# lukecavabarrett/pna

Hardware: NVIDIA H100
Metric: aggregated edges/sec (PNA layer fwd) (higher is better)
Workload: dtype f32

## Files before the change

include/pna_b200.h:

```cpp
#ifndef PNA_B200_H
#define PNA_B200_H

#include <stddef.h>
#include <stdint.h>

#ifdef __cplusplus
extern "C" {
#endif

#define PNA_ABI_VERSION 8

typedef void* pna_stream_t;

enum pna_status {
  PNA_OK = 0,
  PNA_ERR_BAD_ARG = -1,
  PNA_ERR_UNSUPPORTED = -2,
  PNA_ERR_CUDA = -3,
  PNA_ERR_INDEX = -4,
  PNA_ERR_WORKSPACE = -5
};

enum pna_dtype { PNA_F32 = 0, PNA_BF16 = 1 };

enum pna_aggr { PNA_AGGR_SUM = 0, PNA_AGGR_MEAN = 1, PNA_AGGR_MIN = 2, PNA_AGGR_MAX = 3, PNA_AGGR_VAR = 4, PNA_AGGR_STD = 5,
                PNA_AGGR_SKIP = 15  };
enum pna_scaler { PNA_SCALE_IDENTITY = 0, PNA_SCALE_AMPLIFICATION = 1, PNA_SCALE_ATTENUATION = 2, PNA_SCALE_LINEAR = 3, PNA_SCALE_INVERSE_LINEAR = 4 };

#define PNA_MAX_AGGR 6
#define PNA_MAX_SCALERS 5

enum pna_flags {
  PNA_FLAG_ZERO_ISOLATED = 1u,
  PNA_FLAG_SKIP_LIGHT = 2u,
  PNA_FLAG_SKIP_HUBS = 4u,
  PNA_FLAG_GATHER_L1 = 16u,
  PNA_FLAG_RELU_VAR = 8u
};

enum pna_query_what {
  PNA_QUERY_ABI_VERSION = 0,
  PNA_QUERY_SM_ARCH = 1,
  PNA_QUERY_DEFAULT_SPLIT = 2,
  PNA_QUERY_DEFAULT_CHUNK = 3,
  PNA_QUERY_DEVICE_SM_COUNT = 4,
  PNA_QUERY_MAX_FEATURES = 5,
  PNA_QUERY_SIZEOF_CSR = 6,
  PNA_QUERY_SIZEOF_AGG = 7
};

typedef struct pna_csr {
  int64_t n_nodes;
  int64_t n_edges;
  int32_t split_threshold;
  int32_t chunk_edges;
  int32_t* rowptr;
  int32_t* col;
  int32_t* perm;
  int32_t* hub_info;
  int32_t* chunk_items;
  int64_t cap_hubs;
  int64_t cap_chunks;
  int64_t n_hubs;
  int64_t n_chunks;
  int32_t max_degree;
  int32_t n_part;
  int32_t* light_rowptr;
  int32_t* light_deg;
  int32_t* light_col;
  int32_t* part;
// ... 108 lines not shown
```

pna_b200/_lib.py:

```python
from __future__ import annotations

import ctypes as C
import os
import subprocess
import threading

_HERE = os.path.dirname(os.path.abspath(__file__))
REPO_ROOT = os.path.dirname(_HERE)
LIB_PATH = os.environ.get("PNA_B200_LIB") or os.path.join(_HERE, "libpna_sm90.so")
CUDA_SOURCES = [os.path.join(_HERE, "csrc", n) for n in
                ("pna_aggregate.cu", "pna_aggregate_f32_vec.cu", "pna_aggregate_f32_scalar.cu", "pna_aggregate_bf16_vec.cu",
                 "pna_aggregate_bf16_scalar.cu", "pna_aggregate_f32_fsplit.cu", "pna_aggregate_bwd.cu", "pna_linear.cu", "pna_csr.cu", "pna_peer.cu", "pna_misc.cu")]
CUDA_HEADERS = [os.path.join(_HERE, "csrc", n) for n in ("common.cuh", "pna_aggregate.cuh", "pna_aggregate_impl.cuh")] + [
    os.path.join(REPO_ROOT, "include", "pna_b200.h")]
BUILD_DIR = os.path.join(_HERE, "csrc", "build")

NVCC_FLAGS = ["-gencode", "arch=compute_90a,code=sm_90a", "-lineinfo", "-O3", "-std=c++17", "-fmad=false", "-Xcompiler", "-fPIC"]

ABI_VERSION = 8
PNA_OK = 0
PNA_F32, PNA_BF16 = 0, 1
AGGR_CODES = {"sum": 0, "mean": 1, "min": 2, "max": 3, "var": 4, "std": 5, "_skip": 15}
SCALER_CODES = {"identity": 0, "amplification": 1, "attenuation": 2, "linear": 3, "inverse_linear": 4}
FLAG_ZERO_ISOLATED, FLAG_SKIP_LIGHT, FLAG_SKIP_HUBS, FLAG_RELU_VAR, FLAG_GATHER_L1 = 1, 2, 4, 8, 16
(QUERY_ABI_VERSION, QUERY_SM_ARCH, QUERY_DEFAULT_SPLIT, QUERY_DEFAULT_CHUNK, QUERY_DEVICE_SM_COUNT,
 QUERY_MAX_FEATURES, QUERY_SIZEOF_CSR, QUERY_SIZEOF_AGG) = range(8)

EXPORTED_SYMBOLS = ("pna_csr_workspace_bytes", "pna_csr_build", "pna_csr_light_view", "pna_csr_light_view_workspace_bytes", "pna_aggregate_fwd", "pna_aggregate_bwd",
                    "pna_aggregate_bwd_coef", "pna_aggregate_bwd_combine", "pna_aggregate_bwd_slots",
                    "pna_gather_rows", "pna_halo_pull", "pna_halo_grad_pull", "pna_peer_barrier", "pna_linear_fwd", "pna_linear_scaled_fwd", "pna_row_scales", "pna_linear_workspace_bytes", "pna_query", "pna_last_error")


class PnaError(RuntimeError):

    def __init__(self, status: int, message: str):
        super().__init__(f"libpna_sm90 status {status}: {message}")
        self.status = status


class CsrStruct(C.Structure):
    _fields_ = [
        ("n_nodes", C.c_int64), ("n_edges", C.c_int64),
        ("split_threshold", C.c_int32), ("chunk_edges", C.c_int32),
        ("rowptr", C.c_void_p), ("col", C.c_void_p), ("perm", C.c_void_p),
        ("hub_info", C.c_void_p), ("chunk_items", C.c_void_p),
        ("cap_hubs", C.c_int64), ("cap_chunks", C.c_int64),
        ("n_hubs", C.c_int64), ("n_chunks", C.c_int64),
        ("max_degree", C.c_int32), ("n_part", C.c_int32),
        ("light_rowptr", C.c_void_p), ("light_deg", C.c_void_p), ("light_col", C.c_void_p), ("part", C.c_void_p),
        ("n_light_edges", C.c_int64), ("n_src_nodes", C.c_int64), ("hot_source_fraction", C.c_float), ("reserved", C.c_int32),
    ]


class AggStruct(C.Structure):
    _fields_ = [
        ("gathered", C.c_void_p), ("ld_gathered", C.c_int64),
        ("rowptr", C.c_void_p), ("col", C.c_void_p),
# ... 149 lines not shown
```

pna_b200/aggregate.py:

```python
from __future__ import annotations

import ctypes as C
import os
from typing import Mapping, Optional, Sequence, Union

import torch

from . import _lib
from .csr import CSRGraph

_DTYPES = {torch.float32: _lib.PNA_F32, torch.bfloat16: _lib.PNA_BF16}
Names = Union[str, Sequence[str]]


def _names(v: Names) -> list:
    return v.split() if isinstance(v, str) else list(v)


def _ptr(t: Optional[torch.Tensor]):
    return None if t is None else t.data_ptr()


def _rows2d(t: torch.Tensor, what: str) -> torch.Tensor:
    if t.dim() != 2:
        raise ValueError(f"{what} must be 2-D, got shape {tuple(t.shape)}")
    if t.size(1) > 1 and t.stride(1) != 1:
        t = t.contiguous()
    if t.size(0) > 1 and t.stride(0) < t.size(1):
        t = t.contiguous()
    return t


HOT_SOURCE_FRACTION_FOR_L1 = 0.25


DYNAMIC_TAIL_MIN_PARTITION_COST = 256


def _dynamic_tail(csr: CSRGraph) -> bool:
    env = os.environ.get("PNA_B200_DYNAMIC_TAIL")
    if env is not None:
        return env != "0"
    return csr.n_part > 0 and (csr.n_edges + 12 * csr.n_nodes) / csr.n_part >= DYNAMIC_TAIL_MIN_PARTITION_COST


def _check_scaler_degree(t: torch.Tensor, n_rows: int, dev) -> torch.Tensor:
    if t.dtype != torch.int32 or t.device != dev or t.numel() != n_rows or not t.is_contiguous():
        raise ValueError("scaler_degree must be a contiguous int32 [n_rows] tensor on the same device")
    return t


def fold_finalize_enabled() -> bool:
    return os.environ.get("PNA_B200_FOLD_FINALIZE", "0") == "1"


def output_width(n_feat: int, n_aggr: int, n_scalers: int, has_self: bool) -> int:
    return (n_aggr * n_scalers + (1 if has_self else 0)) * n_feat


def aggregate_forward(gathered: torch.Tensor, csr: CSRGraph, aggregators: Names, scalers: Names,
                      avg_deg: Mapping[str, float], *, towers: int = 1, row_bias: Optional[torch.Tensor] = None,
                      self_feat: Optional[torch.Tensor] = None, self_divided: bool = True,
                      messages_in_csr_order: bool = False, zero_isolated: bool = False, relu_var: bool = False,
                      out: Optional[torch.Tensor] = None, row_ids: Optional[torch.Tensor] = None,
                      skip_light: bool = False, skip_hubs: bool = False, view=None, peer=None,
                      scaler_degree: Optional[torch.Tensor] = None, gather_l1: Optional[bool] = None) -> torch.Tensor:
    if not gathered.is_cuda:
        raise ValueError("pna_b200 kernels run on CUDA tensors only; there is no CPU fallback")
    if gathered.dtype not in _DTYPES:
        raise TypeError(f"unsupported dtype {gathered.dtype}; libpna_sm90 takes float32 and bfloat16")
    dev = gathered.device
    if csr.device != dev:
        raise ValueError(f"CSR lives on {csr.device}, features on {dev}")
    gathered = _rows2d(gathered, "gathered")
    F = int(gathered.size(1))
    N = csr.n_nodes
    if F % towers != 0:
        raise ValueError(f"feature width {F} not divisible by towers={towers}")
    Ft = F // towers
    if messages_in_csr_order:
        if gathered.size(0) != csr.n_edges:
            raise ValueError("messages_in_csr_order needs one row per CSR slot")
    n_aggr, aggr_codes = _lib.pack_codes(aggregators, _lib.AGGR_CODES, "aggregator")
    n_scal, scal_codes = _lib.pack_codes(scalers, _lib.SCALER_CODES, "scaler")
    if row_bias is not None:
        row_bias = _rows2d(row_bias.to(gathered.dtype), "row_bias")
        if tuple(row_bias.shape) != (N, F):
            raise ValueError(f"row_bias must be [{N}, {F}]")
    if self_feat is not None:
        self_feat = _rows2d(self_feat.to(gathered.dtype), "self_feat")
        need = F if self_divided else Ft
        if self_feat.size(0) != N or self_feat.size(1) != need:
            raise ValueError(f"self_feat must be [{N}, {need}]")
    width = towers * output_width(Ft, n_aggr, n_scal, self_feat is not None)
    if out is None:
        out = torch.empty((N, width), dtype=gathered.dtype, device=dev)
    else:
        if out.dtype != gathered.dtype or out.device != dev or out.dim() != 2 or out.size(0) != N or out.size(1) < width \
                or out.stride(1) != 1:
            raise ValueError("bad `out` buffer")
    if row_ids is not None:
        if row_ids.dtype != torch.int32 or not row_ids.is_contiguous() or row_ids.device != dev:
            raise ValueError("row_ids must be a contiguous int32 tensor on the same device")
    if gather_l1 is None:
        gather_l1 = (not messages_in_csr_order) and peer is None and csr.hot_source_fraction > HOT_SOURCE_FRACTION_FOR_L1
    flags = (_lib.FLAG_GATHER_L1 if gather_l1 else 0) | \
            (_lib.FLAG_ZERO_ISOLATED if zero_isolated else 0) | (_lib.FLAG_SKIP_LIGHT if skip_light else 0) | \
            (_lib.FLAG_SKIP_HUBS if skip_hubs else 0) | (_lib.FLAG_RELU_VAR if relu_var else 0)
    partials = None if skip_hubs else csr.hub_partials(F)
    d = _lib.AggStruct(
        gathered=_ptr(gathered), ld_gathered=gathered.stride(0) if gathered.size(0) > 1 else F,
        rowptr=_ptr(csr.rowptr), col=None if messages_in_csr_order else (_ptr(csr.col) if csr.n_edges else None),
        row_bias=_ptr(row_bias), ld_row_bias=0 if row_bias is None else (row_bias.stride(0) if N > 1 else F),
        self_feat=_ptr(self_feat), ld_self=0 if self_feat is None else (self_feat.stride(0) if N > 1 else self_feat.size(1)),
        self_tower_stride=Ft if (self_feat is not None and self_divided) else 0,
        out=_ptr(out), ld_out=out.stride(0) if N > 1 else out.size(1),
        n_rows=N, n_feat=F, n_towers=towers, dtype=_DTYPES[gathered.dtype],
        n_aggr=n_aggr, aggr_codes=aggr_codes, n_scalers=n_scal, scaler_codes=scal_codes,
        avg_log=float(avg_deg["log"]), avg_lin=float(avg_deg.get("lin", 1.0)),
        flags=flags, split_threshold=csr.split_threshold, chunk_edges=csr.chunk_edges,
        hub_info=_ptr(csr.hub_info) if csr.n_hubs else None, chunk_items=_ptr(csr.chunk_items) if csr.n_hubs else None,
        n_hubs=csr.n_hubs, n_chunks=csr.n_chunks, hub_partials=_ptr(partials), max_degree=int(csr.max_degree),
        row_ids=_ptr(row_ids), n_row_ids=0 if row_ids is None else int(row_ids.numel()))
    if scaler_degree is not None:
        d.scaler_degree = _check_scaler_degree(scaler_degree, N, dev).data_ptr()
    if view is None and row_ids is None and _dynamic_tail(csr):
        d.work_counter = _ptr(csr.work_counter())
    if view is None and row_ids is None:
        view = csr.full_view()
        if fold_finalize_enabled() and not skip_hubs and peer is None:
            d.hub_done = _ptr(csr.hub_done())
    if view is not None and row_ids is None and N > 0:
        d.light_rowptr, d.light_deg, d.part, d.n_part = _ptr(view.light_rowptr), _ptr(view.light_deg), _ptr(view.part), view.n_part
        d.light_col = _ptr(view.light_col) if csr.n_edges else None
        d.n_view_rows = view.n_view_rows or N
    if peer is not None:
        ptr_table, shift = peer
        if ptr_table.dtype != torch.int64 or ptr_table.device != dev:
            raise ValueError("peer pointer table must be an int64 tensor on the same device")
# ... 186 lines not shown
```

pna_b200/csrc/pna_aggregate_f32_fsplit.cu:

```cuda
#include "pna_aggregate_impl.cuh"

namespace pna {

template <typename Cfg>
static int launch_fsplit(const KParams& p_in, cudaStream_t st) {
  constexpr int VEC = 2, K = 1, DEPTH = 1;
  KParams p = p_in;
  p.n_fpass = (p.F + 32 * VEC * K - 1) / (32 * VEC * K);
  p.work_ctr = nullptr;
  constexpr size_t smem = StreamGeom<float, VEC, K, DEPTH>::kSmem;
  auto kern = k_rows_stream<float, VEC, K, Cfg, false, DEPTH, false>;
  static int resident = 0;
  if (resident == 0) {
    if (smem > 48 * 1024) PNA_CUDA_TRY(cudaFuncSetAttribute(kern, cudaFuncAttributeMaxDynamicSharedMemorySize, (int)smem));
    int dev = 0, sms = 0, nb = 0;
    PNA_CUDA_TRY(cudaGetDevice(&dev));
    PNA_CUDA_TRY(cudaDeviceGetAttribute(&sms, cudaDevAttrMultiProcessorCount, dev));
    PNA_CUDA_TRY(cudaOccupancyMaxActiveBlocksPerMultiprocessor(&nb, kern, kStreamThreads, smem));
    resident = (nb > 0 ? nb : 1) * sms;
  }
  const long long slots = p.n_rows;
  long long gxs = (slots + 8 * (kStreamThreads / 32) - 1) / (8 * (kStreamThreads / 32));
  if (gxs > resident) gxs = resident;
  if (gxs < 1) gxs = 1;
  kern<<<dim3((unsigned)gxs, 1), kStreamThreads, smem, st>>>(p);
  PNA_CUDA_TRY(cudaGetLastError());
  return PNA_OK;
}

int launch_stream_fsplit_f32(const KParams& p, cudaStream_t st) {
  if (p.T != 1 || p.has_self || p.row_ids || (p.F % 64) != 0 || (p.ldx % 2) != 0 || (p.ldo % 2) != 0) return 1;
  return launch_fsplit<CfgMeanMaxMinStd>(p, st);
}

}
```

pna_b200/csrc/pna_aggregate_impl.cuh:

```cuda
#pragma once
#include "pna_aggregate.cuh"
#include <stdlib.h>
#include <string.h>

namespace pna {

constexpr int kThreads = 256;
constexpr int min_blocks(int vec, int k) { return vec * k <= 4 ? 4 : (vec * k <= 8 ? 3 : (vec * k <= 16 ? 2 : 1)); }

template <int VEC>
__device__ __forceinline__ void store_f32(float* p, const float (&v)[VEC]) {
  if constexpr (VEC % 4 == 0) {
#pragma unroll
    for (int i = 0; i < VEC; i += 4) *reinterpret_cast<float4*>(p + i) = make_float4(v[i], v[i + 1], v[i + 2], v[i + 3]);
  } else {
#pragma unroll
    for (int i = 0; i < VEC; ++i) p[i] = v[i];
  }
}

template <typename T, int VEC, int G, int K, int U, typename Cfg>
__global__ void __launch_bounds__(kThreads, min_blocks(VEC, K)) k_rows(const KParams p) {
  constexpr int RPW = 32 / G;
  const int lane = threadIdx.x & 31;
  const int gl = lane % G;
  const long long slot = ((long long)blockIdx.x * (kThreads / 32) + (threadIdx.x >> 5)) * RPW + lane / G;
  long long row;
  if (p.row_ids) {
    if (slot >= p.n_row_ids) return;
    row = __ldg(p.row_ids + slot);
  } else {
    if (slot >= p.n_rows) return;
    row = slot;
  }
  const int beg = __ldg(p.rowptr + row), end = __ldg(p.rowptr + row + 1);
  const int deg = end - beg;
// ... 216 lines not shown
    w[0] = a; w[1] = b; w[2] = c; w[3] = d;
  } else {
    unsigned a, b;
    asm volatile("ld.shared.v2.b32 {%0, %1}, [%2];" : "=r"(a), "=r"(b) : "r"(addr));
    w[0] = a; w[1] = b;
  }
  return r;
}

#ifndef PNA_STREAM_HALF_BYTES
#define PNA_STREAM_HALF_BYTES 4096
#endif
#ifndef PNA_STREAM_STAGES
#define PNA_STREAM_STAGES 2
#endif
template <typename T, int VEC, int K, int DEPTH = 1>
struct StreamGeom {
  static constexpr int kBlockBytes = 32 * VEC * K * (int)sizeof(T);
  static constexpr int kHalf = PNA_STREAM_HALF_BYTES * DEPTH;
  static constexpr int kH = (kHalf / kBlockBytes) < 4 ? 4 : ((kHalf / kBlockBytes) > 32 ? 32 : (kHalf / kBlockBytes));
  static constexpr int kStages = PNA_STREAM_STAGES;
  static constexpr int kWarpBytes = kStages * kH * kBlockBytes;
  static constexpr size_t kSmem = 128 + (size_t)(kStreamThreads / 32) * kWarpBytes;
};

template <bool L1 = false>
__device__ __forceinline__ void cp_async16(unsigned dst, const void* src, unsigned long long policy) {
  if constexpr (L1)
    asm volatile("cp.async.ca.shared.global.L2::cache_hint [%0], [%1], 16, %2;" ::"r"(dst), "l"(__cvta_generic_to_global(src)), "l"(policy)
                 : "memory");
  else
    asm volatile("cp.async.cg.shared.global.L2::cache_hint [%0], [%1], 16, %2;" ::"r"(dst), "l"(__cvta_generic_to_global(src)), "l"(policy)
                 : "memory");
}
__device__ __forceinline__ void cp_async8(unsigned dst, const void* src, unsigned long long policy) {
  asm volatile("cp.async.ca.shared.global.L2::cache_hint [%0], [%1], 8, %2;" ::"r"(dst), "l"(__cvta_generic_to_global(src)), "l"(policy)
               : "memory");
}
template <int BYTES, bool L1 = false>
__device__ __forceinline__ void cp_async_chunk(unsigned dst, const void* src, unsigned long long policy) {
  if constexpr (BYTES == 16) cp_async16<L1>(dst, src, policy); else cp_async8(dst, src, policy);
}
__device__ __forceinline__ void cp_async_commit() { asm volatile("cp.async.commit_group;" ::: "memory"); }
template <int N>
__device__ __forceinline__ void cp_async_wait() { asm volatile("cp.async.wait_group %0;" ::"n"(N) : "memory"); }
__device__ __forceinline__ unsigned long long l2_policy_evict_last() {
  unsigned long long pol;
  asm volatile("createpolicy.fractional.L2::evict_last.b64 %0, 1.0;" : "=l"(pol));
  return pol;
}

#ifndef PNA_STREAM_TMA
#define PNA_STREAM_TMA 0
#endif

constexpr int kFinGroups = 8;

template <int VEC, int K, int UF>
__device__ __forceinline__ void merge_partials(const float* __restrict__ base, long long F, const int (&f)[K], const bool (&ok)[K],
                                               int first, int count, int stride, Acc<VEC> (&acc)[K]) {
  for (int j = 0; j < count; j += UF) {
    float ps[UF][K][4][VEC];
#pragma unroll
    for (int u = 0; u < UF; ++u) {
      if (j + u < count) {
        const float* part = base + (long long)(first + (long long)(j + u) * stride) * 4ll * F;
#pragma unroll
        for (int k = 0; k < K; ++k)
          if (ok[k]) {
#pragma unroll
            for (int q = 0; q < 4; ++q) {
              const float* src = part + (long long)q * F + f[k];
              if constexpr (VEC % 4 == 0) {
#pragma unroll
// ... 47 lines not shown
    if (lane == 0) t = atomicAdd(ctr, 1);
    return __shfl_sync(FULL, t, 0);
  };
  if (nch > kFinGroups) {
    const int g = jc % kFinGroups;
    const int mine = (nch - g + kFinGroups - 1) / kFinGroups;
    if (arrive(cnt + g) != mine - 1) return;
    if (lane == 0) cnt[g] = 0;
    __threadfence();
#pragma unroll
    for (int k = 0; k < K; ++k) acc[k].init();
    merge_partials<VEC, K, UFm>(p.partials, p.F, fm.f, fm.ok, first + g, mine, kFinGroups, acc);
    float* __restrict__ part = p.partials + (long long)(first + g) * 4ll * p.F;
#pragma unroll
    for (int k = 0; k < K; ++k) {
      if (!fm.ok[k]) continue;
      store_f32<VEC>(part + 0ll * p.F + fm.f[k], acc[k].sum);
      store_f32<VEC>(part + 1ll * p.F + fm.f[k], acc[k].sq);
      store_f32<VEC>(part + 2ll * p.F + fm.f[k], acc[k].mn);
      store_f32<VEC>(part + 3ll * p.F + fm.f[k], acc[k].mx);
    }
    if (arrive(cnt + 8) != kFinGroups - 1) return;
  } else if (arrive(cnt + 8) != nch - 1) {
    return;
  }
  if (lane == 0) cnt[8] = 0;
  __threadfence();
#pragma unroll
  for (int k = 0; k < K; ++k) acc[k].init();
  merge_partials<VEC, K, UFm>(p.partials, p.F, fm.f, fm.ok, first, nch > kFinGroups ? kFinGroups : nch, 1, acc);
  finalize_row<T, VEC, G, K, Cfg>(p, fm, (long long)__ldg(p.hub_info + 4 * h), __ldg(p.hub_info + 4 * h + 3), acc);
}

template <typename T, int VEC, int K, typename Cfg, bool BIAS, int DEPTH, bool FOLD = false, bool L1 = false>
__global__ void __launch_bounds__(kStreamThreads, tiled_min_blocks(VEC, K)) k_rows_stream(const __grid_constant__ KParams p) {
  constexpr int G = 32;
  constexpr int H = StreamGeom<T, VEC, K, DEPTH>::kH;
  constexpr int SLOT = StreamGeom<T, VEC, K, DEPTH>::kBlockBytes;
  constexpr int NST = StreamGeom<T, VEC, K, DEPTH>::kStages;
  static_assert(!PNA_STREAM_TMA || NST == 2, "the bulk-copy build variant keeps the two-segment ring");
  constexpr unsigned FULL = 0xffffffffu;
  constexpr bool PEER = DEPTH > 1;
  extern __shared__ __align__(128) unsigned char smem[];
  __shared__ float4 s_scale_lut[kScaleLut];
  const int lane = threadIdx.x & 31;
  const int warp = threadIdx.x >> 5;
  fill_scale_lut(s_scale_lut, p, threadIdx.x, kStreamThreads);

  const unsigned smem0 = smem_u32(smem);
  const unsigned bar0 = smem0 + warp * 16;
  const unsigned ring = smem0 + 128 + warp * StreamGeom<T, VEC, K, DEPTH>::kWarpBytes;
#if PNA_STREAM_TMA
  if (lane == 0) {
    mbar_init(bar0, 1);
    mbar_init(bar0 + 8, 1);
    asm volatile("fence.mbarrier_init.release.cluster;" ::: "memory");
  }
  __syncwarp();
#else
  const unsigned long long keep = l2_policy_evict_last();
  (void)bar0;
#endif

  const long long W = (long long)gridDim.x * (kStreamThreads / 32);
  const long long w = (long long)blockIdx.x * (kStreamThreads / 32) + warp;
  const int n_static = p.work_ctr ? p.n_static : p.n_part;
  int pi_a = (int)((w * n_static) / W), pi_b = (int)(((w + 1) * n_static) / W);
#pragma unroll 1
 for (;;) {
  const int pa = __ldg(p.part + pi_a);
  const int pb = __ldg(p.part + pi_b);
  const int Q0 = __ldg(p.lrowptr + pa);
  const int Te = __ldg(p.lrowptr + pb) - Q0;
  if (pa < pb) {
  const int* __restrict__ lcol = p.lcol + Q0;
  constexpr int CB = VEC * (int)sizeof(T);
  const int n_fpass = p.n_fpass > 1 ? p.n_fpass : 1;
#pragma unroll 1
 for (int fpass = 0; fpass < n_fpass; ++fpass) {
  const int fblock = (blockIdx.y * n_fpass + fpass) * (G * VEC * K);
  const unsigned copy_bytes = (unsigned)(min(G * VEC * K, p.F - fblock) * (int)sizeof(T));
  (void)copy_bytes;
  FeatMap<VEC, G, K> fm;
  fm.init(p, lane, fblock);

#if PNA_STREAM_TMA
  auto source_of = [&](int q) -> int { return (lane < H && q < Te) ? __ldg(lcol + q) : -1; };
#else
  auto source_of = [&](int q) -> int { return (lane < H && q < Te) ? __ldg(lcol + q) : 0; };
#endif
#if PNA_STREAM_TMA
  int tma_issued = 0;
  auto issue_half = [&](int stage, int src) {
    const int nvalid = min(H, Te - tma_issued * H);
    ++tma_issued;
    const unsigned bar = bar0 + stage * 8;
    if (lane == 0) mbar_expect_tx(bar, (unsigned)nvalid * copy_bytes);
    if (src >= 0) bulk_g2s(ring + (stage * H + lane) * SLOT, gathered_row<T>(p, src) + fblock, copy_bytes, bar);
  };
#else
  const int lane_elems = fblock + lane * VEC;
  const char* const xlane = reinterpret_cast<const char*>(static_cast<const T*>(p.x) + lane_elems);
  const unsigned ldxb = (unsigned)p.ldx * (unsigned)sizeof(T);
  auto issue_half = [&](int stage, int src) {
    unsigned dst = ring + (unsigned)(stage * H) * SLOT + lane * CB;
#pragma unroll
    for (int u = 0; u < H; ++u, dst += SLOT) {
      const int s_u = __shfl_sync(FULL, src, u);
      const char* sp;
      if constexpr (PEER) sp = reinterpret_cast<const char*>(gathered_row<T>(p, s_u) + lane_elems);
      else sp = xlane + (unsigned long long)(unsigned)s_u * ldxb;
#pragma unroll
      for (int k = 0; k < K; ++k)
        if (fm.ok[k]) cp_async_chunk<CB, L1>(dst + k * (32 * CB), sp + k * (32 * CB), keep);
    }
    cp_async_commit();
  };
#endif

  int pend = source_of(lane);
  unsigned phase0 = 0, phase1 = 0;
  (void)phase0; (void)phase1;
  if (Te > 0) {
#if PNA_STREAM_TMA
    issue_half(0, pend);
    pend = source_of(H + lane);
    if (H < Te) {
      issue_half(1, pend);
      pend = source_of(2 * H + lane);
    }
#else
#pragma unroll
    for (int s0 = 0; s0 < NST; ++s0) {
      issue_half(s0, pend);
      pend = source_of((s0 + 1) * H + lane);
    }
#endif
  }
  int stage = 0;
  int n_issued = NST;

  auto load_deg = [&](int r) -> int { return (r + lane < pb) ? __ldg(p.ldeg + r + lane) : -1; };
  const ViewMap vmap = {p.n_rows, (int)(p.n_view_rows - p.n_rows)};
  auto load_rid = [&](int r) -> int {
    if (p.row_ids) return (r + lane < pb) ? __ldg(p.row_ids + r + lane) : 0;
    return (int)vmap.to_row(r + lane);
  };
// ... 2 lines not shown
  const unsigned lane_off = (unsigned)lane * (unsigned)CB;
  int q = 0;
#pragma unroll 1
  for (int r0 = pa; r0 < pb; r0 += 32) {
    const int dgN = load_deg(r0 + 32), ridN = load_rid(r0 + 32);
    const int nj = min(32, pb - r0);
#pragma unroll 1
    for (int j = 0; j < nj; ++j) {
      const int deg = __shfl_sync(FULL, dg, j);
      if (deg < 0) continue;
      const int row = __shfl_sync(FULL, rid, j);
      const bool chunk_row = row >= p.n_rows;
      float bias[BIAS ? K : 1][VEC];
      if (BIAS) {
        long long brow = row;
        if (chunk_row) brow = __ldg(p.hub_info + 4 * __ldg(p.chunk_items + 2 * (row - (int)p.n_rows)));
#pragma unroll
        for (int k = 0; k < K; ++k)
          if (fm.ok[k]) Io<T, VEC>::load(static_cast<const T*>(p.bias) + brow * p.ldb + fm.f[k], bias[BIAS ? k : 0]);
      }
      Acc<VEC> acc[K];
#pragma unroll
      for (int k = 0; k < K; ++k) acc[k].init();

      int left = deg;
      while (left > 0) {
        const int inhalf = q & (H - 1);
        if (inhalf == 0) {
#if PNA_STREAM_TMA
          if (stage) { mbar_wait(bar0 + 8, phase1); phase1 ^= 1; }
          else { mbar_wait(bar0, phase0); phase0 ^= 1; }
#else
          cp_async_wait<NST - 1>();
#endif
        }
        const int seg = min(left, H - inhalf);
        unsigned sp = ring + (unsigned)(stage * H + inhalf) * SLOT + lane_off;
        int t = 0;
        for (; t + 2 <= seg; t += 2, sp += 2 * SLOT) {
#pragma unroll
          for (int k = 0; k < K; ++k) {
            if (fm.ok[k]) {
              float m0[VEC], m1[VEC];
              Io<T, VEC>::unpack(lds_raw<T, VEC>(sp + k * (32 * CB)), m0);
              Io<T, VEC>::unpack(lds_raw<T, VEC>(sp + SLOT + k * (32 * CB)), m1);
              acc[k].template add2<BIAS>(m0, m1, bias[BIAS ? k : 0]);
            }
          }
        }
        if (t < seg) {
#pragma unroll
          for (int k = 0; k < K; ++k) {
            if (fm.ok[k]) {
              float m0[VEC];
              Io<T, VEC>::unpack(lds_raw<T, VEC>(sp + k * (32 * CB)), m0);
              acc[k].template add1<BIAS>(m0, bias[BIAS ? k : 0]);
            }
          }
        }
        q += seg;
        left -= seg;
        if ((q & (H - 1)) == 0 || q == Te) {
#if PNA_STREAM_TMA
          __syncwarp();
          if (n_issued * H < Te) {
            issue_half(stage, pend);
            pend = source_of((n_issued + 1) * H + lane);
          }
#else
          issue_half(stage, pend);
          pend = source_of((n_issued + 1) * H + lane);
#endif
          ++n_issued;
          stage = (stage + 1 == NST) ? 0 : stage + 1;
        }
      }
      if (!chunk_row) {
        if (Cfg::kStatic && deg == 0 && !p.sdeg) {
          finalize_isolated_row<T, VEC, G, K, Cfg>(p, fm, (long long)row, scales_of_row(s_scale_lut, p, row, 0));
        } else {
          finalize_row_ds<T, VEC, G, K, Cfg>(p, fm, (long long)row, deg, scales_of_row(s_scale_lut, p, row, deg), acc);
        }
      } else {
        float* __restrict__ part = p.partials + (long long)(row - (int)p.n_rows) * 4ll * p.F;
#pragma unroll
        for (int k = 0; k < K; ++k) {
          if (!fm.ok[k]) continue;
          store_f32<VEC>(part + 0ll * p.F + fm.f[k], acc[k].sum);
          store_f32<VEC>(part + 1ll * p.F + fm.f[k], acc[k].sq);
          store_f32<VEC>(part + 2ll * p.F + fm.f[k], acc[k].mn);
          store_f32<VEC>(part + 3ll * p.F + fm.f[k], acc[k].mx);
        }
        if constexpr (FOLD) fold_split_row<T, VEC, K, Cfg>(p, row - (int)p.n_rows, fblock);
      }
    }
    dg = dgN; rid = ridN;
  }
#if !PNA_STREAM_TMA
  if (n_fpass > 1 || p.work_ctr) { cp_async_wait<0>(); __syncwarp(); }
#endif
 }
  }
// ... 151 lines not shown
  fm.init(p, gl, blockIdx.y * (G * VEC * K));
  Acc<VEC> acc[K];
#pragma unroll
  for (int k = 0; k < K; ++k) acc[k].init();

  const bool two_level = nch > kFinGroups && !p.hub_merged;
  if (p.hub_merged) {
    if (q != 0) return;
    merge_partials<VEC, K, UF>(p.partials, p.F, fm.f, fm.ok, first, 1, 1, acc);
  } else if (two_level) {
    const int mine = (nch - q + kFinGroups - 1) / kFinGroups;
    merge_partials<VEC, K, UF>(p.partials, p.F, fm.f, fm.ok, first + q, mine, kFinGroups, acc);
    float* part = p.partials + (long long)(first + q) * 4ll * p.F;
#pragma unroll
    for (int k = 0; k < K; ++k) {
      if (!fm.ok[k]) continue;
      store_f32<VEC>(part + 0ll * p.F + fm.f[k], acc[k].sum);
      store_f32<VEC>(part + 1ll * p.F + fm.f[k], acc[k].sq);
      store_f32<VEC>(part + 2ll * p.F + fm.f[k], acc[k].mn);
      store_f32<VEC>(part + 3ll * p.F + fm.f[k], acc[k].mx);
    }
    __syncthreads();
    if (q != 0) return;
#pragma unroll
    for (int k = 0; k < K; ++k) acc[k].init();
    merge_partials<VEC, K, UF>(p.partials, p.F, fm.f, fm.ok, first, kFinGroups, 1, acc);
  } else {
    if (q != 0) return;
    merge_partials<VEC, K, UF>(p.partials, p.F, fm.f, fm.ok, first, nch, 1, acc);
  }
  finalize_row<T, VEC, G, K, CfgDynamic>(p, fm, row, deg, acc);
}

int launch_stream_fsplit_f32(const KParams& p, cudaStream_t st);
static inline int feat_split_mode() {
  static int mode = -1;
  if (mode < 0) {
    const char* e = getenv("PNA_B200_FEAT_SPLIT");
    mode = !e ? 0 : (!strcmp(e, "tiled2") ? 1 : (!strcmp(e, "stream2") ? 2 : 0));
  }
  return mode;
}

static inline int stream_oversubscription() {
  static int v = 0;
  if (v == 0) {
    const char* e = getenv("PNA_B200_OVERSUB");
    v = e ? atoi(e) : 1;
    if (v < 1) v = 1;
  }
  return v;
}

template <typename T, int VEC, int G, int K, int U>
static int launch_config(const KParams& p_in, cudaStream_t st) {
  constexpr int RPW = 32 / G;
  constexpr int per_block = (kThreads / 32) * RPW;
  KParams p = p_in;
  const unsigned gy = (unsigned)((p.F + G * VEC * K - 1) / (G * VEC * K));
  if (gy != 1 || !(p.n_view_rows > p.n_rows) || p.hub_merged) p.hub_done = nullptr;
  bool folded = false;
  bool chunks_in_stream = false;
  if (!(p.flags & PNA_FLAG_SKIP_LIGHT)) {
    const long long slots = p.row_ids ? p.n_row_ids : p.n_rows;
    if (slots > 0) {
      const long long gx = (slots + per_block - 1) / per_block;
      PNA_REQUIRE(gx <= 0x7fffffffll, PNA_ERR_UNSUPPORTED, "too many rows for one launch: %lld", slots);
      const unsigned std_s = (0u) | (1u << 4) | (2u << 8);
      const bool s3 = p.nS == 3 && (p.scodes & 0xfffu) == std_s && p.nA == 4;
      const bool s1 = p.nS == 1 && (p.scodes & 0xfu) == PNA_SCALE_IDENTITY && p.nA == 4;
      const int cfg = (p.acodes & 0xffffu) != CfgMeanMaxMinStd::ACODES ? 0 : s3 ? 1 : s1 ? 2 : 0;
      bool fsplit_done = false;
      if constexpr (G == 32 && VEC == 4 && K == 1 && sizeof(T) == 4) {
        if (feat_split_mode() == 2 && p.lrowptr != nullptr && p.col != nullptr && p.peer_x == nullptr && p.bias == nullptr &&
            cfg == 1 && p.F == 128) {
          p.hub_done = nullptr;
          const int rc = launch_stream_fsplit_f32(p, st);
          if (rc < 0) return rc;
          fsplit_done = rc == 0;
          if (fsplit_done) chunks_in_stream = p.n_view_rows > p.n_rows;
        }
      }
      if (fsplit_done) {
      } else if (G == 32 && VEC > 1 && p.lrowptr != nullptr && p.col != nullptr) {
       if constexpr (G == 32 && VEC > 1) {
        const bool b = p.bias != nullptr;
        const bool deep = p.peer_x != nullptr;
#define PNA_LAUNCH_STREAM_(CFG, B, DEPTH, FOLD) PNA_LAUNCH_STREAM__(CFG, B, DEPTH, FOLD, false)
#define PNA_LAUNCH_STREAM__(CFG, B, DEPTH, FOLD, L1)                                                                    \
  do {                                                                                                             \
    constexpr size_t smem = StreamGeom<T, VEC, K, DEPTH>::kSmem;                                                   \
    auto kern = k_rows_stream<T, VEC, K, CFG, B, DEPTH, FOLD, L1>;                                                     \
    static int resident = 0;                  \
    if (resident == 0) {                                                                                           \
      if (smem > 48 * 1024) PNA_CUDA_TRY(cudaFuncSetAttribute(kern, cudaFuncAttributeMaxDynamicSharedMemorySize, (int)smem)); \
      int dev = 0, sms = 0, nb = 0;                                                                                \
      PNA_CUDA_TRY(cudaGetDevice(&dev));                                                                           \
      PNA_CUDA_TRY(cudaDeviceGetAttribute(&sms, cudaDevAttrMultiProcessorCount, dev));                             \
      PNA_CUDA_TRY(cudaOccupancyMaxActiveBlocksPerMultiprocessor(&nb, kern, kStreamThreads, smem));                \
      resident = (nb > 0 ? nb : 1) * sms;                                                                          \
    }                                                                                                              \
    long long gxs = (slots + 8 * (kStreamThreads / 32) - 1) / (8 * (kStreamThreads / 32));  \
    if (gxs > (long long)resident * stream_oversubscription()) gxs = (long long)resident * stream_oversubscription(); \
    if (gxs < 1) gxs = 1;                                                                                          \
    if (p.work_ctr) {     \
      const long long nw = gxs * (kStreamThreads / 32);                                                            \
      p.n_static = (int)((long long)p.n_part * 7 / 10);                                                            \
      if (gy != 1 || p.n_static < nw || gxs < resident) p.work_ctr = nullptr;                                      \
      else PNA_CUDA_TRY(cudaMemsetAsync(p.work_ctr, 0, sizeof(int), st));                                          \
    }                                                                                                              \
    kern<<<dim3((unsigned)gxs, gy), kStreamThreads, smem, st>>>(p);                                                \
  } while (0)
#define PNA_LAUNCH_STREAM(CFG, B)                                        \
  do {                                                                   \
    if (p.hub_done) PNA_LAUNCH_STREAM_(CFG, B, 1, true);                 \
    else PNA_LAUNCH_STREAM_(CFG, B, 1, false);                           \
// ... 44 lines not shown
  if (!(p.flags & PNA_FLAG_SKIP_HUBS) && p.n_hubs > 0) {
    if (!chunks_in_stream) {
      const long long gc = (p.n_chunks + per_block - 1) / per_block;
      k_hub_chunks<T, VEC, G, K, U><<<dim3((unsigned)gc, gy), kThreads, 0, st>>>(p);
      PNA_CUDA_TRY(cudaGetLastError());
    }
    if (!folded) {
      if constexpr (G == 32) {
        if (p.hub_merged) {
          for (long long S = 1; S < p.n_chunks; S *= kTreeR) {
            const long long blocks = (p.n_chunks + kTreeR * S - 1) / (kTreeR * S);
            k_hub_tree<VEC, K><<<dim3((unsigned)((blocks + 3) / 4), gy), 128, 0, st>>>(p, S);
            PNA_CUDA_TRY(cudaGetLastError());
          }
        }
      } else {
        p.hub_merged = 0;
      }
      k_hub_finalize<T, VEC, G, K><<<dim3((unsigned)p.n_hubs, gy), kFinGroups * G, 0, st>>>(p);
      PNA_CUDA_TRY(cudaGetLastError());
    }
  }
  return PNA_OK;
}

template <typename T, int VEC>
int launch_typed(const KParams& p, cudaStream_t st) {
  const int chunks = p.F / VEC;
  if (chunks <= 1) return launch_config<T, VEC, 1, 1, 4>(p, st);
  if (chunks <= 2) return launch_config<T, VEC, 2, 1, 4>(p, st);
  if (chunks <= 4) return launch_config<T, VEC, 4, 1, 4>(p, st);
  if (chunks <= 8) return launch_config<T, VEC, 8, 1, 4>(p, st);
  if (chunks <= 16) return launch_config<T, VEC, 16, 1, 4>(p, st);
  if (chunks == 32 && feat_split_mode() == 1) return launch_config<T, VEC, 16, 1, 4>(p, st);
  if (chunks <= 32) return launch_config<T, VEC, 32, 1, 4>(p, st);
  if (chunks <= 64) return launch_config<T, VEC, 32, 2, 2>(p, st);
  if (chunks <= 96) return launch_config<T, VEC, 32, 3, 2>(p, st);
  return launch_config<T, VEC, 32, 4, 2>(p, st);
}

}
```

Measured before the change: 1.939 billion.

## Add L2-sized feature-slab mode for f32 PNA stream aggregation

```diff
diff --git a/include/pna_b200.h b/include/pna_b200.h
--- a/include/pna_b200.h
+++ b/include/pna_b200.h
@@ -35,7 +35,8 @@
   PNA_FLAG_SKIP_LIGHT = 2u,
   PNA_FLAG_SKIP_HUBS = 4u,
   PNA_FLAG_GATHER_L1 = 16u,
-  PNA_FLAG_RELU_VAR = 8u
+  PNA_FLAG_RELU_VAR = 8u,
+  PNA_FLAG_FEATURE_SLAB = 32u
 };
 
 enum pna_query_what {
diff --git a/pna_b200/_lib.py b/pna_b200/_lib.py
--- a/pna_b200/_lib.py
+++ b/pna_b200/_lib.py
@@ -10,7 +10,7 @@
 LIB_PATH = os.environ.get("PNA_B200_LIB") or os.path.join(_HERE, "libpna_sm90.so")
 CUDA_SOURCES = [os.path.join(_HERE, "csrc", n) for n in
                 ("pna_aggregate.cu", "pna_aggregate_f32_vec.cu", "pna_aggregate_f32_scalar.cu", "pna_aggregate_bf16_vec.cu",
-                 "pna_aggregate_bf16_scalar.cu", "pna_aggregate_f32_fsplit.cu", "pna_aggregate_bwd.cu", "pna_linear.cu", "pna_csr.cu", "pna_peer.cu", "pna_misc.cu")]
+                 "pna_aggregate_bf16_scalar.cu", "pna_aggregate_bwd.cu", "pna_linear.cu", "pna_csr.cu", "pna_peer.cu", "pna_misc.cu")]
 CUDA_HEADERS = [os.path.join(_HERE, "csrc", n) for n in ("common.cuh", "pna_aggregate.cuh", "pna_aggregate_impl.cuh")] + [
     os.path.join(REPO_ROOT, "include", "pna_b200.h")]
 BUILD_DIR = os.path.join(_HERE, "csrc", "build")
@@ -23,6 +23,7 @@
 AGGR_CODES = {"sum": 0, "mean": 1, "min": 2, "max": 3, "var": 4, "std": 5, "_skip": 15}
 SCALER_CODES = {"identity": 0, "amplification": 1, "attenuation": 2, "linear": 3, "inverse_linear": 4}
 FLAG_ZERO_ISOLATED, FLAG_SKIP_LIGHT, FLAG_SKIP_HUBS, FLAG_RELU_VAR, FLAG_GATHER_L1 = 1, 2, 4, 8, 16
+FLAG_FEATURE_SLAB = 32
 (QUERY_ABI_VERSION, QUERY_SM_ARCH, QUERY_DEFAULT_SPLIT, QUERY_DEFAULT_CHUNK, QUERY_DEVICE_SM_COUNT,
  QUERY_MAX_FEATURES, QUERY_SIZEOF_CSR, QUERY_SIZEOF_AGG) = range(8)
 
diff --git a/pna_b200/aggregate.py b/pna_b200/aggregate.py
--- a/pna_b200/aggregate.py
+++ b/pna_b200/aggregate.py
@@ -54,6 +54,32 @@
     return os.environ.get("PNA_B200_FOLD_FINALIZE", "0") == "1"
 
 
+FEATURE_SLAB_COLUMNS = 64
+FEATURE_SLAB_L2_FRACTION = 1.0
+_SLAB_AGGR_CODES = 1 | 3 << 4 | 2 << 8 | 5 << 12
+_SLAB_SCALER_CODES = {3: 0 | 1 << 4 | 2 << 8, 1: 0}
+
+
+def feature_slab_columns(n_src: int, n_feat: int, elem_size: int, l2_bytes: int, eligible: bool = True) -> int:
+    cols = FEATURE_SLAB_COLUMNS
+    if not eligible or elem_size != 4 or n_feat <= cols or n_feat % cols != 0:
+        return 0
+    budget = FEATURE_SLAB_L2_FRACTION * l2_bytes
+    if n_src * n_feat * elem_size <= budget or n_src * cols * elem_size > budget:
+        return 0
+    return cols
+
+
+_L2_BYTES: dict = {}
+
+
+def _l2_bytes(dev: torch.device) -> int:
+    idx = dev.index if dev.index is not None else torch.cuda.current_device()
+    if idx not in _L2_BYTES:
+        _L2_BYTES[idx] = int(torch.cuda.get_device_properties(idx).L2_cache_size)
+    return _L2_BYTES[idx]
+
+
 def output_width(n_feat: int, n_aggr: int, n_scalers: int, has_self: bool) -> int:
     return (n_aggr * n_scalers + (1 if has_self else 0)) * n_feat
 
@@ -64,7 +90,8 @@
                       messages_in_csr_order: bool = False, zero_isolated: bool = False, relu_var: bool = False,
                       out: Optional[torch.Tensor] = None, row_ids: Optional[torch.Tensor] = None,
                       skip_light: bool = False, skip_hubs: bool = False, view=None, peer=None,
-                      scaler_degree: Optional[torch.Tensor] = None, gather_l1: Optional[bool] = None) -> torch.Tensor:
+                      scaler_degree: Optional[torch.Tensor] = None, gather_l1: Optional[bool] = None,
+                      feature_slab: Optional[int] = None) -> torch.Tensor:
     if not gathered.is_cuda:
         raise ValueError("pna_b200 kernels run on CUDA tensors only; there is no CPU fallback")
     if gathered.dtype not in _DTYPES:
@@ -104,7 +131,14 @@
             raise ValueError("row_ids must be a contiguous int32 tensor on the same device")
     if gather_l1 is None:
         gather_l1 = (not messages_in_csr_order) and peer is None and csr.hot_source_fraction > HOT_SOURCE_FRACTION_FOR_L1
-    flags = (_lib.FLAG_GATHER_L1 if gather_l1 else 0) | \
+    if feature_slab is None:
+        eligible = (not messages_in_csr_order and row_bias is None and peer is None and row_ids is None and not gather_l1
+                    and n_aggr == 4 and (aggr_codes & 0xffff) == _SLAB_AGGR_CODES
+                    and _SLAB_SCALER_CODES.get(n_scal) == scal_codes)
+        feature_slab = feature_slab_columns(int(gathered.size(0)), F, gathered.element_size(), _l2_bytes(dev), eligible)
+    if feature_slab not in (0, FEATURE_SLAB_COLUMNS):
+        raise ValueError(f"feature_slab must be None, 0 or {FEATURE_SLAB_COLUMNS}, got {feature_slab!r}")
+    flags = (_lib.FLAG_FEATURE_SLAB if feature_slab else 0) | (_lib.FLAG_GATHER_L1 if gather_l1 else 0) | \
             (_lib.FLAG_ZERO_ISOLATED if zero_isolated else 0) | (_lib.FLAG_SKIP_LIGHT if skip_light else 0) | \
             (_lib.FLAG_SKIP_HUBS if skip_hubs else 0) | (_lib.FLAG_RELU_VAR if relu_var else 0)
     partials = None if skip_hubs else csr.hub_partials(F)
diff --git a/pna_b200/csrc/pna_aggregate_f32_fsplit.cu b/pna_b200/csrc/pna_aggregate_f32_fsplit.cu
--- a/pna_b200/csrc/pna_aggregate_f32_fsplit.cu
+++ /dev/null
@@ -1,36 +0,0 @@
-#include "pna_aggregate_impl.cuh"
-
-namespace pna {
-
-template <typename Cfg>
-static int launch_fsplit(const KParams& p_in, cudaStream_t st) {
-  constexpr int VEC = 2, K = 1, DEPTH = 1;
-  KParams p = p_in;
-  p.n_fpass = (p.F + 32 * VEC * K - 1) / (32 * VEC * K);
-  p.work_ctr = nullptr;
-  constexpr size_t smem = StreamGeom<float, VEC, K, DEPTH>::kSmem;
-  auto kern = k_rows_stream<float, VEC, K, Cfg, false, DEPTH, false>;
-  static int resident = 0;
-  if (resident == 0) {
-    if (smem > 48 * 1024) PNA_CUDA_TRY(cudaFuncSetAttribute(kern, cudaFuncAttributeMaxDynamicSharedMemorySize, (int)smem));
-    int dev = 0, sms = 0, nb = 0;
-    PNA_CUDA_TRY(cudaGetDevice(&dev));
-    PNA_CUDA_TRY(cudaDeviceGetAttribute(&sms, cudaDevAttrMultiProcessorCount, dev));
-    PNA_CUDA_TRY(cudaOccupancyMaxActiveBlocksPerMultiprocessor(&nb, kern, kStreamThreads, smem));
-    resident = (nb > 0 ? nb : 1) * sms;
-  }
-  const long long slots = p.n_rows;
-  long long gxs = (slots + 8 * (kStreamThreads / 32) - 1) / (8 * (kStreamThreads / 32));
-  if (gxs > resident) gxs = resident;
-  if (gxs < 1) gxs = 1;
-  kern<<<dim3((unsigned)gxs, 1), kStreamThreads, smem, st>>>(p);
-  PNA_CUDA_TRY(cudaGetLastError());
-  return PNA_OK;
-}
-
-int launch_stream_fsplit_f32(const KParams& p, cudaStream_t st) {
-  if (p.T != 1 || p.has_self || p.row_ids || (p.F % 64) != 0 || (p.ldx % 2) != 0 || (p.ldo % 2) != 0) return 1;
-  return launch_fsplit<CfgMeanMaxMinStd>(p, st);
-}
-
-}
diff --git a/pna_b200/csrc/pna_aggregate_impl.cuh b/pna_b200/csrc/pna_aggregate_impl.cuh
--- a/pna_b200/csrc/pna_aggregate_impl.cuh
+++ b/pna_b200/csrc/pna_aggregate_impl.cuh
@@ -1,7 +1,6 @@
 #pragma once
 #include "pna_aggregate.cuh"
 #include <stdlib.h>
-#include <string.h>
 
 namespace pna {
 
@@ -284,14 +283,6 @@
   else
     asm volatile("cp.async.cg.shared.global.L2::cache_hint [%0], [%1], 16, %2;" ::"r"(dst), "l"(__cvta_generic_to_global(src)), "l"(policy)
                  : "memory");
-}
-__device__ __forceinline__ void cp_async8(unsigned dst, const void* src, unsigned long long policy) {
-  asm volatile("cp.async.ca.shared.global.L2::cache_hint [%0], [%1], 8, %2;" ::"r"(dst), "l"(__cvta_generic_to_global(src)), "l"(policy)
-               : "memory");
-}
-template <int BYTES, bool L1 = false>
-__device__ __forceinline__ void cp_async_chunk(unsigned dst, const void* src, unsigned long long policy) {
-  if constexpr (BYTES == 16) cp_async16<L1>(dst, src, policy); else cp_async8(dst, src, policy);
 }
 __device__ __forceinline__ void cp_async_commit() { asm volatile("cp.async.commit_group;" ::: "memory"); }
 template <int N>
@@ -405,13 +396,18 @@
   finalize_row<T, VEC, G, K, Cfg>(p, fm, (long long)__ldg(p.hub_info + 4 * h), __ldg(p.hub_info + 4 * h + 3), acc);
 }
 
-template <typename T, int VEC, int K, typename Cfg, bool BIAS, int DEPTH, bool FOLD = false, bool L1 = false>
+template <typename T, int VEC, int K, typename Cfg, bool BIAS, int DEPTH, bool FOLD = false, bool L1 = false, int SB = 0>
 __global__ void __launch_bounds__(kStreamThreads, tiled_min_blocks(VEC, K)) k_rows_stream(const __grid_constant__ KParams p) {
   constexpr int G = 32;
   constexpr int H = StreamGeom<T, VEC, K, DEPTH>::kH;
   constexpr int SLOT = StreamGeom<T, VEC, K, DEPTH>::kBlockBytes;
   constexpr int NST = StreamGeom<T, VEC, K, DEPTH>::kStages;
   static_assert(!PNA_STREAM_TMA || NST == 2, "the bulk-copy build variant keeps the two-segment ring");
+  static_assert(SB == 0 || (SB == 256 && SLOT == SB && K == 1 && sizeof(T) == 4 && !BIAS && DEPTH == 1 && !FOLD && !L1 &&
+                            !PNA_STREAM_TMA),
+                "slab mode: fp32 256-byte slabs, one slab-row per ring slot, no bias / peers / folded finalize / L1 copies");
+  constexpr int CPS = SB > 0 ? SB / 16 : 1;
+  constexpr int SPC = 32 / CPS;
   constexpr unsigned FULL = 0xffffffffu;
   constexpr bool PEER = DEPTH > 1;
   extern __shared__ __align__(128) unsigned char smem[];
@@ -472,20 +468,29 @@
     if (src >= 0) bulk_g2s(ring + (stage * H + lane) * SLOT, gathered_row<T>(p, src) + fblock, copy_bytes, bar);
   };
 #else
-  const int lane_elems = fblock + lane * VEC;
+  const int lane_elems = fblock + (SB > 0 ? (lane % CPS) * (16 / (int)sizeof(T)) : lane * VEC);
   const char* const xlane = reinterpret_cast<const char*>(static_cast<const T*>(p.x) + lane_elems);
   const unsigned ldxb = (unsigned)p.ldx * (unsigned)sizeof(T);
   auto issue_half = [&](int stage, int src) {
-    unsigned dst = ring + (unsigned)(stage * H) * SLOT + lane * CB;
-#pragma unroll
-    for (int u = 0; u < H; ++u, dst += SLOT) {
-      const int s_u = __shfl_sync(FULL, src, u);
-      const char* sp;
-      if constexpr (PEER) sp = reinterpret_cast<const char*>(gathered_row<T>(p, s_u) + lane_elems);
-      else sp = xlane + (unsigned long long)(unsigned)s_u * ldxb;
-#pragma unroll
-      for (int k = 0; k < K; ++k)
-        if (fm.ok[k]) cp_async_chunk<CB, L1>(dst + k * (32 * CB), sp + k * (32 * CB), keep);
+    if constexpr (SB > 0) {
+      unsigned dst = ring + (unsigned)(stage * H + lane / CPS) * SLOT + (lane % CPS) * 16;
+#pragma unroll
+      for (int u = 0; u < H; u += SPC, dst += SPC * SLOT) {
+        const int s_u = __shfl_sync(FULL, src, u + lane / CPS);
+        cp_async16<false>(dst, xlane + (unsigned long long)(unsigned)s_u * ldxb, keep);
+      }
+    } else {
+      unsigned dst = ring + (unsigned)(stage * H) * SLOT + lane * CB;
+#pragma unroll
+      for (int u = 0; u < H; ++u, dst += SLOT) {
+        const int s_u = __shfl_sync(FULL, src, u);
+        const char* sp;
+        if constexpr (PEER) sp = reinterpret_cast<const char*>(gathered_row<T>(p, s_u) + lane_elems);
+        else sp = xlane + (unsigned long long)(unsigned)s_u * ldxb;
+#pragma unroll
+        for (int k = 0; k < K; ++k)
+          if (fm.ok[k]) cp_async16<L1>(dst + k * (32 * CB), sp + k * (32 * CB), keep);
+      }
     }
     cp_async_commit();
   };
@@ -554,11 +559,22 @@
           else { mbar_wait(bar0, phase0); phase0 ^= 1; }
 #else
           cp_async_wait<NST - 1>();
+          if constexpr (SB > 0) __syncwarp();
 #endif
         }
         const int seg = min(left, H - inhalf);
         unsigned sp = ring + (unsigned)(stage * H + inhalf) * SLOT + lane_off;
         int t = 0;
+        if constexpr (SB > 0) {
+          constexpr int SU = 8 / VEC;
+          for (; t + SU <= seg; t += SU, sp += SU * SLOT) {
+            float m[SU][VEC];
+#pragma unroll
+            for (int u = 0; u < SU; ++u) Io<T, VEC>::unpack(lds_raw<T, VEC>(sp + u * SLOT), m[u]);
+#pragma unroll
+            for (int u = 0; u < SU; u += 2) acc[0].template add2<false>(m[u], m[u + 1], bias[0]);
+          }
+        }
         for (; t + 2 <= seg; t += 2, sp += 2 * SLOT) {
 #pragma unroll
           for (int k = 0; k < K; ++k) {
@@ -590,6 +606,7 @@
             pend = source_of((n_issued + 1) * H + lane);
           }
 #else
+          if constexpr (SB > 0) __syncwarp();
           issue_half(stage, pend);
           pend = source_of((n_issued + 1) * H + lane);
 #endif
@@ -807,16 +824,6 @@
   finalize_row<T, VEC, G, K, CfgDynamic>(p, fm, row, deg, acc);
 }
 
-int launch_stream_fsplit_f32(const KParams& p, cudaStream_t st);
-static inline int feat_split_mode() {
-  static int mode = -1;
-  if (mode < 0) {
-    const char* e = getenv("PNA_B200_FEAT_SPLIT");
-    mode = !e ? 0 : (!strcmp(e, "tiled2") ? 1 : (!strcmp(e, "stream2") ? 2 : 0));
-  }
-  return mode;
-}
-
 static inline int stream_oversubscription() {
   static int v = 0;
   if (v == 0) {
@@ -825,6 +832,36 @@
     if (v < 1) v = 1;
   }
   return v;
+}
+
+static inline bool slab_mode(const KParams& p, int cfg) {
+  return (p.flags & PNA_FLAG_FEATURE_SLAB) && p.lrowptr != nullptr && p.col != nullptr && p.bias == nullptr && p.peer_x == nullptr &&
+         p.row_ids == nullptr && !(p.flags & PNA_FLAG_GATHER_L1) && (cfg == 1 || cfg == 2) && p.F % 64 == 0;
+}
+
+template <typename Cfg>
+static int launch_slab(const KParams& p_in, long long slots, cudaStream_t st) {
+  constexpr int SB = 256, VEC = SB / 128;
+  KParams p = p_in;
+  p.n_fpass = p.F / (SB / 4);
+  p.work_ctr = nullptr;
+  p.hub_done = nullptr;
+  constexpr size_t smem = StreamGeom<float, VEC, 1, 1>::kSmem;
+  auto kern = k_rows_stream<float, VEC, 1, Cfg, false, 1, false, false, SB>;
+  static int resident = 0;
+  if (resident == 0) {
+    if (smem > 48 * 1024) PNA_CUDA_TRY(cudaFuncSetAttribute(kern, cudaFuncAttributeMaxDynamicSharedMemorySize, (int)smem));
+    int dev = 0, sms = 0, nb = 0;
+    PNA_CUDA_TRY(cudaGetDevice(&dev));
+    PNA_CUDA_TRY(cudaDeviceGetAttribute(&sms, cudaDevAttrMultiProcessorCount, dev));
+    PNA_CUDA_TRY(cudaOccupancyMaxActiveBlocksPerMultiprocessor(&nb, kern, kStreamThreads, smem));
+    resident = (nb > 0 ? nb : 1) * sms;
+  }
+  long long gxs = (slots + 8 * (kStreamThreads / 32) - 1) / (8 * (kStreamThreads / 32));
+  if (gxs > (long long)resident * stream_oversubscription()) gxs = (long long)resident * stream_oversubscription();
+  if (gxs < 1) gxs = 1;
+  kern<<<dim3((unsigned)gxs, 1), kStreamThreads, smem, st>>>(p);
+  return PNA_OK;
 }
 
 template <typename T, int VEC, int G, int K, int U>
@@ -845,18 +882,14 @@
       const bool s3 = p.nS == 3 && (p.scodes & 0xfffu) == std_s && p.nA == 4;
       const bool s1 = p.nS == 1 && (p.scodes & 0xfu) == PNA_SCALE_IDENTITY && p.nA == 4;
       const int cfg = (p.acodes & 0xffffu) != CfgMeanMaxMinStd::ACODES ? 0 : s3 ? 1 : s1 ? 2 : 0;
-      bool fsplit_done = false;
-      if constexpr (G == 32 && VEC == 4 && K == 1 && sizeof(T) == 4) {
-        if (feat_split_mode() == 2 && p.lrowptr != nullptr && p.col != nullptr && p.peer_x == nullptr && p.bias == nullptr &&
-            cfg == 1 && p.F == 128) {
-          p.hub_done = nullptr;
-          const int rc = launch_stream_fsplit_f32(p, st);
-          if (rc < 0) return rc;
-          fsplit_done = rc == 0;
-          if (fsplit_done) chunks_in_stream = p.n_view_rows > p.n_rows;
-        }
-      }
-      if (fsplit_done) {
+      bool slab = false;
+      if constexpr (sizeof(T) == 4 && VEC == 4) slab = slab_mode(p, cfg);
+      if (slab) {
+        if constexpr (sizeof(T) == 4 && VEC == 4) {
+          const int rc = cfg == 1 ? launch_slab<CfgMeanMaxMinStd>(p, slots, st) : launch_slab<CfgMeanMaxMinStdId>(p, slots, st);
+          if (rc != PNA_OK) return rc;
+          chunks_in_stream = p.n_view_rows > p.n_rows;
+        }
       } else if (G == 32 && VEC > 1 && p.lrowptr != nullptr && p.col != nullptr) {
        if constexpr (G == 32 && VEC > 1) {
         const bool b = p.bias != nullptr;
@@ -967,7 +1000,6 @@
   if (chunks <= 4) return launch_config<T, VEC, 4, 1, 4>(p, st);
   if (chunks <= 8) return launch_config<T, VEC, 8, 1, 4>(p, st);
   if (chunks <= 16) return launch_config<T, VEC, 16, 1, 4>(p, st);
-  if (chunks == 32 && feat_split_mode() == 1) return launch_config<T, VEC, 16, 1, 4>(p, st);
   if (chunks <= 32) return launch_config<T, VEC, 32, 1, 4>(p, st);
   if (chunks <= 64) return launch_config<T, VEC, 32, 2, 2>(p, st);
   if (chunks <= 96) return launch_config<T, VEC, 32, 3, 2>(p, st);
```

After: 2.023 billion (median of 6 runs). 1.04x the previous value.
